# zhuwsh/ORB-SLAM2

Measured on AMD Instinct MI355X. Metric: frames/sec ORB extract+match, 1241x376 @1000 feats; bit-exact vs CPU, higher is better.
Workload: dtype u8; 1 GPU; KITTI-shape stereo 1241x376, nFeatures=1000/eye, 8 levels, FAST 20/7: extract(L)+extract(R)+ComputeStereoMatches; 1 frame = 1 stereo pair; images RESIDENT IN HBM when the timed region starts (kernel throughput: excludes PCIe; fed from pinned host memory the same path runs at config.host_fed_batched_frames_per_s -- the PCIe Gen5 x16 link, 0.96 MB per frame -- and one camera stream at config.host_fe; parallelism=1 independent camera-stream batches, one per GPU, ranks_seen=1, backend=none

## Files before the change

### orb-slam2_amd/csrc/orbx_stereo.hip

```cpp
#include "orbx_device.h"
#include <stdlib.h>
#include <algorithm>

struct StereoTabs {
    float sf[ORBX_MAX_LEVELS]; float isf[ORBX_MAX_LEVELS];
    unsigned long long reach_pk;
};

__device__ __forceinline__ int lvl_px(const uint8_t *img, int pitch, int w, int h, int x, int y)
{
    return img[(long long)reflect101(y, h) * pitch + reflect101(x, w)];
}

template <bool FOLD>
__device__ __forceinline__ void st_store(Published<float> u_right, Published<float> depth, Published<int> st_dist, long long og, float u, float z, int sad)
{
    if (FOLD) { u_right.put(og, u); depth.put(og, z); st_dist.put(og, sad); }
    else {
        u_right.plain_across_launches()[og] = u; depth.plain_across_launches()[og] = z; st_dist.plain_across_launches()[og] = sad;
    }
}

extern __shared__ __align__(16) int prep_smem[];

__global__ __launch_bounds__(256) void k_stereo_prep(const Geom *__restrict__ g, const orbx_keypoint *__restrict__ kR,
                                                     const int *__restrict__ nR, int cap, StereoTabs tabs,
                                                     int *__restrict__ row_off, uint4 *__restrict__ entries, int ent_cap)
{
    __shared__ int s_w[4];
    const int p = blockIdx.x, tid = threadIdx.x;
    const int rows = g->lv[0].h, n_r = min(nR[p], ent_cap);
    int *cnt = prep_smem, *cur = prep_smem + ((rows + 4) & ~3);
    const orbx_keypoint *kr = kR + (long long)p * cap;
    for (int i = tid; i < rows; i += 256) { cnt[i] = 0; cur[i] = 0; }
    __syncthreads();
    for (int ir = tid; ir < n_r; ir += 256) atomicAdd(&cnt[min(max((int)floorf(kr[ir].y), 0), rows - 1)], 1);
    __syncthreads();
    const int total = lds_excl_scan(cnt, rows, s_w);
    int *ro = row_off + (long long)p * (rows + 1);
    for (int i = tid; i < rows; i += 256) ro[i] = cnt[i];
    if (tid == 0) ro[rows] = total;
    uint4 *en = entries + (long long)p * ent_cap;
    for (int ir = tid; ir < n_r; ir += 256) {
        const orbx_keypoint q = kr[ir];
        const float y = q.y, r = 2.0f * tabs.sf[q.octave & (ORBX_MAX_LEVELS - 1)];
        const int maxr = min((int)ceilf(y + r), rows - 1), minr = max((int)floorf(y - r), 0);
        const int c = min(max((int)floorf(y), 0), rows - 1);
        en[cnt[c] + atomicAdd(&cur[c], 1)] = make_uint4((unsigned)ir | ((unsigned)q.octave << 16), __float_as_uint(q.x),
                                                        (unsigned)minr | ((unsigned)maxr << 16), 0u);
    }
}

__device__ __forceinline__ void hist_select(const int *hist, int k, int *sel, int *rem)
{
    const int lane = threadIdx.x;
    const int4 v = reinterpret_cast<const int4 *>(hist)[lane];
    const int s = v.x + v.y + v.z + v.w, inc = wave_incl_scan(s);
    const unsigned long long m = __ballot(inc > k);
    const int L = m ? __builtin_ctzll(m) : 63;
    if (lane == L) {
        int acc = inc - s, b = 0;
        if (acc + v.x > k) b = 0;
        else if (acc + v.x + v.y > k) { b = 1; acc += v.x; }
        else if (acc + v.x + v.y + v.z > k) { b = 2; acc += v.x + v.y; }
        else { b = 3; acc += v.x + v.y + v.z; }
        *sel = 4 * L + b; *rem = k - acc;
    }
}

__device__ __forceinline__ void stereo_cut(int n_l, long long o, Published<float> u_right, Published<float> depth, Published<int> st_dist)
{
    __shared__ __align__(16) int hist[256];
    __shared__ int s_sel, s_rem, s_cnt;
    const int tid = threadIdx.x;
    constexpr int K = 8;
    int d[K];
#pragma unroll
    for (int k = 0; k < K; k++) {
        const int i = tid + 256 * k;
        d[k] = i < n_l ? st_dist.get(o + i) : -1;
    }
    hist[tid] = 0;
    if (tid == 0) s_cnt = 0;
    __syncthreads();
    int local = 0;
#pragma unroll
    for (int k = 0; k < K; k++) if (d[k] >= 0) { atomicAdd(&hist[d[k] >> 8], 1); local++; }
    for (int i = tid + 256 * K; i < n_l; i += 256) {
        const int v = st_dist.get(o + i);
        if (v >= 0) { atomicAdd(&hist[v >> 8], 1); local++; }
    }
    if (local) atomicAdd(&s_cnt, local);
    __syncthreads();
    const int nvd = s_cnt;
    if (nvd == 0) return;
    if (tid < 64) hist_select(hist, nvd / 2, &s_sel, &s_rem);
    __syncthreads();
    const int hi = s_sel, rem = s_rem;
    __syncthreads();
    hist[tid] = 0;
    __syncthreads();
#pragma unroll
    for (int k = 0; k < K; k++) if (d[k] >= 0 && (d[k] >> 8) == hi) atomicAdd(&hist[d[k] & 255], 1);
    for (int i = tid + 256 * K; i < n_l; i += 256) {
        const int v = st_dist.get(o + i);
        if (v >= 0 && (v >> 8) == hi) atomicAdd(&hist[v & 255], 1);
    }
    __syncthreads();
    if (tid < 64) hist_select(hist, rem, &s_sel, &s_rem);
    __syncthreads();
    const float median = (float)((hi << 8) | s_sel);
    const float th_dist = 1.5f * 1.4f * median;
#pragma unroll
    for (int k = 0; k < K; k++)
        if (d[k] >= 0 && !((float)d[k] < th_dist)) { u_right.put(o + tid + 256 * k, -1.0f); depth.put(o + tid + 256 * k, -1.0f); }
    for (int i = tid + 256 * K; i < n_l; i += 256) {
        const int v = st_dist.get(o + i);
        if (v >= 0 && !((float)v < th_dist)) { u_right.put(o + i, -1.0f); depth.put(o + i, -1.0f); }
    }
}

#ifndef STX_G
#define STX_G 16
#endif
template <bool FOLD>
__global__ __launch_bounds__(256) __attribute__((amdgpu_waves_per_eu(8, 8))) void k_stereo(const Geom *__restrict__ g, PyrRef prL, PyrRef prR, int img_l0, int img_r0,
                                                const orbx_keypoint *__restrict__ kL, const uint32_t *__restrict__ dL,
                                                const int *__restrict__ nL, const orbx_keypoint *__restrict__ kR,
                                                const uint32_t *__restrict__ dR, const int *__restrict__ nR, int cap,
                                                float bf, float max_d, StereoTabs tabs, Published<float> u_right,
                                                Published<float> depth, Published<int> st_dist,
                                                const int *__restrict__ row_off, const uint4 *__restrict__ entries, int ent_cap, int reach,
                                                int *__restrict__ arrive, int kpw, int xmap_gx, int xmap_pairs)
{
    constexpr int SW_BYTES = 11 * 16 + 11 * 28 + 4;
    __shared__ __align__(16) uint8_t s_win[4 * ((SW_BYTES + 15) & ~15)];
    int p, bx;
    if (xmap_gx > 0) {
        const unsigned L = blockIdx.x, slot = L >> 3, per = (unsigned)xmap_gx * STX_G, grp = slot / per, rem = slot - grp * per;
        bx = (int)(rem / STX_G); p = (int)((grp * STX_G + rem % STX_G) * 8u + (L & 7u));
        if (p >= xmap_pairs) return;
    } else { p = blockIdx.y; bx = blockIdx.x; }
    const int lane = threadIdx.x & 63, sub = lane >> 4, sl = lane & 15;
    const int il_base = (bx * 4 + (threadIdx.x >> 6)) * kpw;
    const int n_l = nL[p];
    if (bx * 4 * kpw >= n_l) return;
    if (il_base < n_l) {
    const int il = il_base + sub;
    const bool have = il < n_l && sub < kpw;
    const long long ol = (long long)p * cap + (have ? il : il_base);
    const uint32_t *dr = dR + (long long)p * cap * 8;
    const orbx_keypoint kp = kL[ol];
    const int level_l = min(max(kp.octave, 0), g->nlevels - 1);
    const float vl = kp.y, ul = kp.x;
    const int n_rows = g->lv[0].h;
    const int row = (int)vl;
    const float min_u = ul - max_d, max_u = ul;
    const bool active = have && row >= 0 && row < n_rows && !(max_u < 0);
    unsigned mine = 0xFFFFFFFFu;
    float mine_x = 0.f;
    {
        uint32_t a[8];
#pragma unroll
        for (int i = 0; i < 8; i++) a[i] = dL[ol * 8 + i];
        const int *ro = row_off + (long long)p * (n_rows + 1);
        const uint4 *en = entries + (long long)p * ent_cap;
        const int rl = (int)((tabs.reach_pk >> (4 * level_l)) & 15ull);
        const int rch = rl == 15 ? reach : min(reach, rl);
        const int b0 = active ? ro[max(row - rch, 0)] : 0, e1 = active ? ro[min(row + rch, n_rows - 1) + 1] : 0;
        for (int base = b0; __any(base < e1); base += 16) {
            const int j = base + sl;
            if (j < e1) {
                const uint4 ent = en[j];
                const int ir = (int)(ent.x & 0xFFFFu), oct = (int)(short)(ent.x >> 16);
                const float qx = __uint_as_float(ent.y);
                const int minr = (int)(ent.z & 0xFFFFu), maxr = (int)(ent.z >> 16);
                if (row >= minr && row <= maxr && oct >= level_l - 1 && oct <= level_l + 1 && qx >= min_u && qx <= max_u) {
                    uint32_t bq[8];
                    const uint4 *src = reinterpret_cast<const uint4 *>(dr + (long long)ir * 8);
                    const uint4 v0 = src[0], v1 = src[1];
                    bq[0] = v0.x; bq[1] = v0.y; bq[2] = v0.z; bq[3] = v0.w;
                    bq[4] = v1.x; bq[5] = v1.y; bq[6] = v1.z; bq[7] = v1.w;
                    const int dist = hamming256(a, bq);
                    if (dist < 100) {
                        const unsigned key = ((unsigned)dist << 16) | (unsigned)ir;
                        if (key < mine) { mine = key; mine_x = qx; }
                    }
                }
            }
        }
    }
    const unsigned best_row = row16_min_u32(mine);
    const unsigned bx_row = row16_or_u32(mine == best_row && mine != 0xFFFFFFFFu ? __float_as_uint(mine_x) : 0u);
    for (int gk = 0; gk < kpw; gk++) {
        if (il_base + gk >= n_l) break;
        const unsigned best = (unsigned)__builtin_amdgcn_readlane((int)best_row, gk * 16);
        const int best_dist = best == 0xFFFFFFFFu ? 100 : (int)(best >> 16);
        const float ur0 = __uint_as_float((unsigned)__builtin_amdgcn_readlane((int)bx_row, gk * 16));
        const float kx = __uint_as_float((unsigned)__builtin_amdgcn_readlane((int)__float_as_uint(kp.x), gk * 16));
        const float ky = __uint_as_float((unsigned)__builtin_amdgcn_readlane((int)__float_as_uint(kp.y), gk * 16));
        const int lvl = __builtin_amdgcn_readlane(level_l, gk * 16);
        const long long og = (long long)p * cap + il_base + gk;
        if (!(best_dist < 75)) {
            if (lane == 0) st_store<FOLD>(u_right, depth, st_dist, og, -1.0f, -1.0f, -1);
            continue;
        }
        float out_u = -1.0f, out_z = -1.0f;
        int out_sad = -1;
        const float sfac = tabs.isf[lvl];
        const float sul = roundf(kx * sfac), svl = roundf(ky * sfac), sur0 = roundf(ur0 * sfac);
        const LevelGeom &LV = g->lv[lvl];
        const float iniu = sur0 + 5 - 5, endu = sur0 + 5 + 5 + 1;
        if (!(iniu < 0 || endu >= (float)LV.w)) {
            int pl, prr;
            const uint8_t *imL = orbx_level_ptr(prL, LV, lvl, img_l0 + p, &pl);
            const uint8_t *imR = orbx_level_ptr(prR, LV, lvl, img_r0 + p, &prr);
            const int cy = (int)svl, cxl = (int)sul;
            const int e0 = lane, e1 = lane + 64 < 121 ? lane + 64 : 60;
            const int dy0 = e0 / 11 - 5, dx0 = e0 % 11 - 5;
            const int dy1 = e1 / 11 - 5, dx1 = e1 % 11 - 5;
            const int cx0 = (int)sur0;
            int lc, il0, il1, r0[11], r1[11];
            const bool inside = cy - 5 >= 0 && cy + 5 < LV.h && cxl - 5 >= 0 && cxl + 5 < LV.w && cx0 - 10 >= 0 && cx0 + 10 < LV.w &&
                                ((((uintptr_t)imL | (uintptr_t)imR | (unsigned)pl | (unsigned)prr) & 3) == 0);
            if (inside) {
                uint8_t *wl = s_win + (threadIdx.x >> 6) * ((SW_BYTES + 15) & ~15), *wr = wl + 11 * 16;
                const int xla = (cxl - 5) & ~3, xra = (cx0 - 10) & ~3;
                uint32_t vr0, vr1 = 0, vlw = 0;
                {
                    const int rr = lane / 7, cc = lane - rr * 7;
                    const int xo_ = min(xra + 4 * cc, (prr - 4));
                    vr0 = *reinterpret_cast<const uint32_t *>(imR + (long long)(cy - 5 + rr) * prr + xo_);
                    if (lane < 13) {
                        const int i2 = lane + 64, r2 = i2 / 7, c2 = i2 - r2 * 7;
                        vr1 = *reinterpret_cast<const uint32_t *>(imR + (long long)(cy - 5 + r2) * prr + min(xra + 4 * c2, prr - 4));
                    }
                    if (lane < 44) {
                        const int r3 = lane >> 2, c3 = lane & 3;
                        vlw = *reinterpret_cast<const uint32_t *>(imL + (long long)(cy - 5 + r3) * pl + min(xla + 4 * c3, pl - 4));
                    }
                    __builtin_amdgcn_wave_barrier();
                    reinterpret_cast<uint32_t *>(wr)[lane] = vr0;
                    if (lane < 13) reinterpret_cast<uint32_t *>(wr)[lane + 64] = vr1;
                    if (lane < 44) reinterpret_cast<uint32_t *>(wl)[lane] = vlw;
                }
                __builtin_amdgcn_fence(__ATOMIC_RELEASE, "wavefront");
                __builtin_amdgcn_wave_barrier();
                const int ol_ = cxl - xla, or_ = cx0 - xra;
                typedef const volatile __attribute__((address_space(3))) uint8_t *lds_bytes;
                const lds_bytes vl_ = (lds_bytes)wl, vr_ = (lds_bytes)wr;
                lc = vl_[5 * 16 + ol_];
                il0 = vl_[(dy0 + 5) * 16 + ol_ + dx0];
                il1 = vl_[(dy1 + 5) * 16 + ol_ + dx1];
#pragma unroll
                for (int k = 0; k < 11; k++) {
                    r0[k] = vr_[(dy0 + 5) * 28 + or_ + dx0 + k - 5];
                    r1[k] = vr_[(dy1 + 5) * 28 + or_ + dx1 + k - 5];
                }
                asm volatile("" : "+v"(lc), "+v"(il0), "+v"(il1));
#pragma unroll
                for (int k = 0; k < 11; k++) asm volatile("" : "+v"(r0[k]), "+v"(r1[k]));
            } else {
                lc = lvl_px(imL, pl, LV.w, LV.h, cxl, cy);
                il0 = lvl_px(imL, pl, LV.w, LV.h, cxl + dx0, cy + dy0);
                il1 = lvl_px(imL, pl, LV.w, LV.h, cxl + dx1, cy + dy1);
#pragma unroll
                for (int k = 0; k < 11; k++) {
                    r0[k] = lvl_px(imR, prr, LV.w, LV.h, cx0 + dx0 + k - 5, cy + dy0);
                    r1[k] = lvl_px(imR, prr, LV.w, LV.h, cx0 + dx1 + k - 5, cy + dy1);
                }
            }
            int dists[11];
            unsigned lpk = (unsigned)il0 | ((unsigned)il1 << 16), lcc = (unsigned)lc * 0x00010001u;
            asm volatile("" : "+v"(lcc));
            auto shift_sad = [&](int k) -> unsigned {
                const unsigned rc = (unsigned)__builtin_amdgcn_readlane(r0[k], 60) * 0x00010001u;
                const unsigned rpk = (unsigned)r0[k] | ((unsigned)r1[k] << 16);
                return __builtin_amdgcn_sad_u16(lpk + rc, rpk + lcc, 0u);
            };
#pragma unroll
            for (int k = 0; k < 11; k += 2) {
                const unsigned sa = shift_sad(k);
                if (k + 1 < 11) {
                    const unsigned sb = shift_sad(k + 1);
                    const unsigned tot = (unsigned)wave_sum((int)(sa | (sb << 16)));
                    dists[k] = (int)(tot & 0xFFFFu);
                    dists[k + 1] = (int)(tot >> 16);
                } else {
                    dists[k] = wave_sum((int)sa);
                }
            }
            int best_sad = 0x7FFFFFFF, best_inc = 0;
#pragma unroll
            for (int k = 0; k < 11; k++)
                if (dists[k] < best_sad) { best_sad = dists[k]; best_inc = k - 5; }
            if (!(best_inc == -5 || best_inc == 5)) {
                float d1 = 0, d2 = 0, d3 = 0;
#pragma unroll
                for (int k = 1; k < 10; k++)
                    if (k == best_inc + 5) { d1 = (float)dists[k - 1]; d2 = (float)dists[k]; d3 = (float)dists[k + 1]; }
                const float delta = (d1 - d3) / (2.0f * (d1 + d3 - 2.0f * d2));
                if (!(delta < -1 || delta > 1)) {
                    float best_ur = tabs.sf[lvl] * ((float)sur0 + (float)best_inc + delta);
                    float disparity = kx - best_ur;
                    if (disparity >= 0 && disparity < max_d) {
                        if (disparity <= 0) { disparity = 0.01f; best_ur = (float)((double)kx - 0.01); }
                        out_z = bf / disparity;
                        out_u = best_ur;
                        out_sad = best_sad;
                    }
                }
            }
        }
        if (lane == 0) st_store<FOLD>(u_right, depth, st_dist, og, out_u, out_z, out_sad);
    }
    }
    if (!FOLD) return;
    __shared__ int s_last;
    publish_drain();
    __syncthreads();
    if (threadIdx.x == 0) {
        const int nwg = (n_l + 4 * kpw - 1) / (4 * kpw);
        const int old = publish_arrive(&arrive[p]);
        s_last = old == nwg - 1;
        if (old == nwg - 1) __hip_atomic_store(&arrive[p], 0, __ATOMIC_RELAXED, __HIP_MEMORY_SCOPE_AGENT);
    }
    __syncthreads();
    if (!s_last) return;
    stereo_cut(n_l, (long long)p * cap, u_right, depth, st_dist);
}

__global__ __launch_bounds__(256) void k_stereo_cut(const int *__restrict__ nL, int cap, Published<float> u_right,
                                                    Published<float> depth, Published<int> st_dist)
{
    stereo_cut(nL[blockIdx.x], (long long)blockIdx.x * cap, u_right, depth, st_dist);
}

static int same_geometry(const orbx_extractor *L, const orbx_extractor *R)
{
    if (L->nlevels != R->nlevels || L->geom.w != R->geom.w || L->geom.h != R->geom.h || L->geom.w == 0) return 0;
    for (int i = 0; i < L->nlevels; i++) if (L->sf[i] != R->sf[i]) return 0;
    return 1;
}

extern "C" int orbx_stereo_row_table_available(const orbx_extractor *R, const void *d_kR, int img_r0, int batch, int cap)
{
    return R && d_kR && img_r0 >= 0 && batch >= 1 && R->d_rt_off && R->rt_kps && cap == R->rt_cap && img_r0 + batch <= R->rt_batch &&
           (const char *)d_kR == (const char *)R->rt_kps + (size_t)img_r0 * cap * sizeof(orbx_keypoint);
}

extern "C" int orbx_stereo_match_batch_device(orbx_extractor *L, int img_l0, orbx_extractor *R, int img_r0, int batch,
                                              const void *d_kL, const void *d_dL, const void *d_nL,
                                              const void *d_kR, const void *d_dR, const void *d_nR, int cap,
                                              float bf, float min_z, void *d_u_right, void *d_depth, int row_table, void *stream)
{
    if (row_table != ORBX_ROWTAB_FROM_KEYPOINTS && row_table != ORBX_ROWTAB_OF_EXTRACTION) { orbx_set_error("row_table: unknown source %d", row_table); return ORBX_E_INVALID; }
    if (!L || !R || !d_kL || !d_dL || !d_nL || !d_kR || !d_dR || !d_nR || !d_u_right || !d_depth || batch < 1 || cap < 1 ||
        img_l0 < 0 || img_r0 < 0 || img_l0 + batch > L->last_batch || img_r0 + batch > R->last_batch || !(min_z > 0)) {
        orbx_set_error("orbx_stereo_match_batch_device: invalid argument");
        return ORBX_E_INVALID;
    }
    if (L->device != R->device || !same_geometry(L, R)) {
        orbx_set_error("left and right extractors differ in device, image size or scale tables");
        return ORBX_E_INVALID;
    }
    if (cap >= 65536) { orbx_set_error("cap must be < 65536"); return ORBX_E_INVALID; }
    ORBX_HIP(orbx_use_device(L->device));
    hipStream_t s = stream ? (hipStream_t)stream : L->stream;
    const size_t need = (size_t)batch * cap * sizeof(int);
    if (need > L->st_cap || !L->d_st_dist) {
        ORBX_HIP(hipStreamSynchronize(s));
        { const int qrc = orbx_quiesce(L); if (qrc) return qrc; }
        { const int erc = ensure(&L->d_st_dist, &L->st_cap, need); if (erc) return erc; }
    }
    StereoTabs tabs;
    tabs.reach_pk = 0;
    for (int i = 0; i < ORBX_MAX_LEVELS; i++) {
        tabs.sf[i] = L->sf[i]; tabs.isf[i] = L->isf[i];
        const int rl = (int)ceilf(2.0f * L->sf[std::min(i + 1, L->nlevels - 1)]) + 1;
        tabs.reach_pk |= (unsigned long long)std::min(rl, 15) << (4 * i);
    }
    const int rows = L->geom.lv[0].h;
    const int ent_cap = cap;
    const int reach = (int)ceilf(2.0f * L->sf[L->nlevels - 1]) + 1;
    void *d_row_off, *d_entries;
    int row_ent_cap = ent_cap;
    const bool by_product = row_table == ORBX_ROWTAB_OF_EXTRACTION;
    if (by_product && !orbx_stereo_row_table_available(R, d_kR, img_r0, batch, cap)) {
        orbx_set_error("ORBX_ROWTAB_OF_EXTRACTION: the right handle's last extraction left no row table for this keypoint buffer / capacity / image range");
        return ORBX_E_INVALID;
    }
    if (by_product) {
        d_row_off = R->d_rt_off + (size_t)img_r0 * (rows + 1);
        d_entries = R->d_rt_entries + (size_t)img_r0 * R->rt_ent_cap * sizeof(uint4);
        row_ent_cap = R->rt_ent_cap;
    } else {
        int rc;
        if ((rc = orbx_scratch(L, 7, (size_t)batch * (rows + 1) * sizeof(int), &d_row_off))) return rc;
        const size_t need_e = (size_t)batch * ent_cap * sizeof(uint4);
        if (need_e > L->st_ent_cap || !L->d_st_entries) {
            ORBX_HIP(hipStreamSynchronize(s));
            { const int qrc = orbx_quiesce(L); if (qrc) return qrc; }
            if ((rc = ensure(&L->d_st_entries, &L->st_ent_cap, need_e))) return rc;
        }
        d_entries = L->d_st_entries;
    }
    PyrRef pl, pr;
    pl.img0 = L->last_img0; pl.img0_stride = (long long)L->last_img_stride; pl.img0_pitch = (int)L->last_pitch;
    pl.pyr = L->d_pyr; pl.pyr_stride = L->geom.pyr_bytes;
    pr.img0 = R->last_img0; pr.img0_stride = (long long)R->last_img_stride; pr.img0_pitch = (int)R->last_pitch;
    pr.pyr = R->d_pyr; pr.pyr_stride = R->geom.pyr_bytes;
    { int urc = orbx_use_stream(L, s); if (urc) return urc; if (R != L && (urc = orbx_use_stream(R, s))) return urc; }
    const float max_d = bf / min_z;
    if (!L->d_st_arrive) {
        ORBX_HIP(hipMalloc((void **)&L->d_st_arrive, (size_t)L->max_batch * sizeof(int)));
        ORBX_HIP(hipMemsetAsync(L->d_st_arrive, 0, (size_t)L->max_batch * sizeof(int), s));
    }
    orbx_prof_begin(L, ORBX_STAGE_STEREO, s);
    if (!by_product)
        hipLaunchKernelGGL(k_stereo_prep, dim3(batch), dim3(256), (size_t)2 * ((rows + 4) & ~3) * sizeof(int), s, L->d_geom,
                           (const orbx_keypoint *)d_kR, (const int *)d_nR, cap, tabs, (int *)d_row_off, (uint4 *)d_entries, ent_cap);
    const int kpw_forced = L->stereo_kpw_forced;
    const int kpw = kpw_forced ? kpw_forced : (long long)batch * cap <= 2560 ? 1 : 4;
    const bool fold = kpw == 1;
    const int gx = (cap + 4 * kpw - 1) / (4 * kpw);
#ifdef STX_NOXMAP
    const bool xmap = false;
#else
    const bool xmap = !fold && batch >= 16 && (long long)gx * ((batch + 8 * STX_G - 1) / (8 * STX_G)) * 8 * STX_G < (1ll << 30);
#endif
    const dim3 grid = xmap ? dim3((unsigned)(gx * ((batch + 8 * STX_G - 1) / (8 * STX_G)) * 8 * STX_G)) : dim3(gx, batch);
    L->last_forms[7] = kpw; L->last_forms[8] = xmap;
    hipLaunchKernelGGL((fold ? k_stereo<true> : k_stereo<false>), grid, dim3(256), 0, s, L->d_geom, pl, pr, img_l0, img_r0,
                       (const orbx_keypoint *)d_kL, (const uint32_t *)d_dL, (const int *)d_nL,
                       (const orbx_keypoint *)d_kR, (const uint32_t *)d_dR, (const int *)d_nR, cap, bf, max_d, tabs,
                       Published<float>((float *)d_u_right), Published<float>((float *)d_depth), Published<int>(L->d_st_dist), (const int *)d_row_off, (const uint4 *)d_entries, row_ent_cap, reach,
                       L->d_st_arrive, kpw, xmap ? gx : 0, batch);
    if (!fold) hipLaunchKernelGGL(k_stereo_cut, dim3(batch), dim3(256), 0, s, (const int *)d_nL, cap, Published<float>((float *)d_u_right), Published<float>((float *)d_depth), Published<int>(L->d_st_dist));
    orbx_prof_end(L, s);
    ORBX_HIP(hipGetLastError());
    return ORBX_OK;
}

extern "C" int orbx_stereo_match(orbx_extractor *L, orbx_extractor *R,
                                 const orbx_keypoint *kL, const uint8_t *dL, int nL,
                                 const orbx_keypoint *kR, const uint8_t *dR, int nR,
                                 float bf, float min_z, float *u_right, float *depth)
{
    if (!L || !R || nL < 0 || nR < 0 || (nL && (!kL || !dL || !u_right || !depth)) || (nR && (!kR || !dR))) {
        orbx_set_error("orbx_stereo_match: invalid argument");
        return ORBX_E_INVALID;
    }
    if (nL == 0) return ORBX_OK;
    for (int i = 0; i < nL; i++)
        if (kL[i].octave < 0 || kL[i].octave >= L->nlevels) { orbx_set_error("left keypoint %d: octave %d out of range", i, kL[i].octave); return ORBX_E_INVALID; }
    for (int i = 0; i < nR; i++)
        if (kR[i].octave < 0 || kR[i].octave >= L->nlevels) { orbx_set_error("right keypoint %d: octave %d out of range", i, kR[i].octave); return ORBX_E_INVALID; }
    if (!L->last_img0 || !R->last_img0) { orbx_set_error("run orbx_extract on both eyes first"); return ORBX_E_INVALID; }
    ORBX_HIP(orbx_use_device(L->device));
    ORBX_HIP(hipStreamSynchronize(R->stream));
    const int cap = nL > nR ? nL : (nR > 0 ? nR : 1);
    void *bkL, *bdL, *bkR, *bdR, *bn, *bu, *bz;
    int rc;
    if ((rc = orbx_scratch(L, 0, sizeof(orbx_keypoint) * cap, &bkL)) || (rc = orbx_scratch(L, 1, 32 * (size_t)cap, &bdL)) ||
        (rc = orbx_scratch(L, 2, sizeof(orbx_keypoint) * cap, &bkR)) || (rc = orbx_scratch(L, 3, 32 * (size_t)cap, &bdR)) ||
        (rc = orbx_scratch(L, 4, 2 * sizeof(int), &bn)) || (rc = orbx_scratch(L, 5, 4 * (size_t)cap, &bu)) ||
        (rc = orbx_scratch(L, 6, 4 * (size_t)cap, &bz)))
        return rc;
    const int counts[2] = { nL, nR };
    hipStream_t s = L->stream;
    ORBX_HIP(hipMemcpyAsync(bkL, kL, sizeof(orbx_keypoint) * nL, hipMemcpyHostToDevice, s));
    ORBX_HIP(hipMemcpyAsync(bdL, dL, 32 * (size_t)nL, hipMemcpyHostToDevice, s));
    if (nR) {
        ORBX_HIP(hipMemcpyAsync(bkR, kR, sizeof(orbx_keypoint) * nR, hipMemcpyHostToDevice, s));
        ORBX_HIP(hipMemcpyAsync(bdR, dR, 32 * (size_t)nR, hipMemcpyHostToDevice, s));
    }
    ORBX_HIP(hipMemcpyAsync(bn, counts, sizeof counts, hipMemcpyHostToDevice, s));
    L->prof_chain = false;
    rc = orbx_stereo_match_batch_device(L, 0, R, 0, 1, bkL, bdL, bn, bkR, bdR, (int *)bn + 1, cap, bf, min_z, bu, bz, ORBX_ROWTAB_FROM_KEYPOINTS, s);
    if (rc) return rc;
    ORBX_HIP(hipMemcpyAsync(u_right, bu, 4 * (size_t)nL, hipMemcpyDeviceToHost, s));
    ORBX_HIP(hipMemcpyAsync(depth, bz, 4 * (size_t)nL, hipMemcpyDeviceToHost, s));
    ORBX_HIP(hipStreamSynchronize(s));
    return ORBX_OK;
}
```

Baseline: 159,500 frames/s.

## Prefetch stereo SAD windows for all per-wave keypoints via async global-to-LDS loads

Result: no change. 159,800 frames/s (median of 5 runs) (+0.2%).

```diff
diff --git a/orb-slam2_amd/csrc/orbx_stereo.hip b/orb-slam2_amd/csrc/orbx_stereo.hip
--- a/orb-slam2_amd/csrc/orbx_stereo.hip
+++ b/orb-slam2_amd/csrc/orbx_stereo.hip
@@ -123,6 +123,8 @@
 #ifndef STX_G
 #define STX_G 16
 #endif
+constexpr int STX_SLOT = (11 * 16 + 11 * 28 + 4 + 15) & ~15;
+extern __shared__ __align__(16) uint8_t stereo_smem[];
 template <bool FOLD>
 __global__ __launch_bounds__(256) __attribute__((amdgpu_waves_per_eu(8, 8))) void k_stereo(const Geom *__restrict__ g, PyrRef prL, PyrRef prR, int img_l0, int img_r0,
                                                 const orbx_keypoint *__restrict__ kL, const uint32_t *__restrict__ dL,
@@ -131,10 +133,10 @@
                                                 float bf, float max_d, StereoTabs tabs, Published<float> u_right,
                                                 Published<float> depth, Published<int> st_dist,
                                                 const int *__restrict__ row_off, const uint4 *__restrict__ entries, int ent_cap, int reach,
-                                                int *__restrict__ arrive, int kpw, int xmap_gx, int xmap_pairs)
-{
-    constexpr int SW_BYTES = 11 * 16 + 11 * 28 + 4;
-    __shared__ __align__(16) uint8_t s_win[4 * ((SW_BYTES + 15) & ~15)];
+                                                int *__restrict__ arrive, int kpw_arg, int xmap_gx, int xmap_pairs)
+{
+    constexpr int kpw = FOLD ? 1 : 4;
+    (void)kpw_arg;
     int p, bx;
     if (xmap_gx > 0) {
         const unsigned L = blockIdx.x, slot = L >> 3, per = (unsigned)xmap_gx * STX_G, grp = slot / per, rem = slot - grp * per;
@@ -168,85 +170,119 @@
         const int rl = (int)((tabs.reach_pk >> (4 * level_l)) & 15ull);
         const int rch = rl == 15 ? reach : min(reach, rl);
         const int b0 = active ? ro[max(row - rch, 0)] : 0, e1 = active ? ro[min(row + rch, n_rows - 1) + 1] : 0;
-        for (int base = b0; __any(base < e1); base += 16) {
-            const int j = base + sl;
-            if (j < e1) {
-                const uint4 ent = en[j];
-                const int ir = (int)(ent.x & 0xFFFFu), oct = (int)(short)(ent.x >> 16);
-                const float qx = __uint_as_float(ent.y);
-                const int minr = (int)(ent.z & 0xFFFFu), maxr = (int)(ent.z >> 16);
-                if (row >= minr && row <= maxr && oct >= level_l - 1 && oct <= level_l + 1 && qx >= min_u && qx <= max_u) {
-                    uint32_t bq[8];
-                    const uint4 *src = reinterpret_cast<const uint4 *>(dr + (long long)ir * 8);
-                    const uint4 v0 = src[0], v1 = src[1];
-                    bq[0] = v0.x; bq[1] = v0.y; bq[2] = v0.z; bq[3] = v0.w;
-                    bq[4] = v1.x; bq[5] = v1.y; bq[6] = v1.z; bq[7] = v1.w;
-                    const int dist = hamming256(a, bq);
-                    if (dist < 100) {
-                        const unsigned key = ((unsigned)dist << 16) | (unsigned)ir;
-                        if (key < mine) { mine = key; mine_x = qx; }
-                    }
-                }
+        for (int base = b0; __any(base < e1); base += 32) {
+            const int j0 = base + sl, j1 = j0 + 16;
+            uint4 ent0 = make_uint4(0u, 0u, 0u, 0u), ent1 = ent0;
+            if (j0 < e1) ent0 = en[j0];
+            if (j1 < e1) ent1 = en[j1];
+            const int ir0 = (int)(ent0.x & 0xFFFFu), oct0 = (int)(short)(ent0.x >> 16), ir1 = (int)(ent1.x & 0xFFFFu), oct1 = (int)(short)(ent1.x >> 16);
+            const float qx0 = __uint_as_float(ent0.y), qx1 = __uint_as_float(ent1.y);
+            const int minr0 = (int)(ent0.z & 0xFFFFu), maxr0 = (int)(ent0.z >> 16), minr1 = (int)(ent1.z & 0xFFFFu), maxr1 = (int)(ent1.z >> 16);
+            const bool ok0 = j0 < e1 && row >= minr0 && row <= maxr0 && oct0 >= level_l - 1 && oct0 <= level_l + 1 && qx0 >= min_u && qx0 <= max_u;
+            const bool ok1 = j1 < e1 && row >= minr1 && row <= maxr1 && oct1 >= level_l - 1 && oct1 <= level_l + 1 && qx1 >= min_u && qx1 <= max_u;
+            uint4 p0 = make_uint4(0u, 0u, 0u, 0u), p1 = p0, q0 = p0, q1 = p0;
+            if (ok0) { const uint4 *src = reinterpret_cast<const uint4 *>(dr + (long long)ir0 * 8); p0 = src[0]; p1 = src[1]; }
+            if (ok1) { const uint4 *src = reinterpret_cast<const uint4 *>(dr + (long long)ir1 * 8); q0 = src[0]; q1 = src[1]; }
+            const uint32_t bp[8] = { p0.x, p0.y, p0.z, p0.w, p1.x, p1.y, p1.z, p1.w }, bq[8] = { q0.x, q0.y, q0.z, q0.w, q1.x, q1.y, q1.z, q1.w };
+            const int dist0 = hamming256(a, bp), dist1 = hamming256(a, bq);
+            if (ok0 && dist0 < 100) {
+                const unsigned key = ((unsigned)dist0 << 16) | (unsigned)ir0;
+                if (key < mine) { mine = key; mine_x = qx0; }
+            }
+            if (ok1 && dist1 < 100) {
+                const unsigned key = ((unsigned)dist1 << 16) | (unsigned)ir1;
+                if (key < mine) { mine = key; mine_x = qx1; }
             }
         }
     }
     const unsigned best_row = row16_min_u32(mine);
     const unsigned bx_row = row16_or_u32(mine == best_row && mine != 0xFFFFFFFFu ? __float_as_uint(mine_x) : 0u);
+    struct Fine {
+        bool match, range, inside;
+        int lvl, w, h, cy, cxl, cx0;
+        float kx, sur0;
+    };
+    struct FineImgs { const uint8_t *imL, *imR; int pl, prr; };
+    auto imgs_of = [&](int lvl) -> FineImgs {
+        FineImgs m;
+        const LevelGeom &LV = g->lv[lvl];
+        m.imL = orbx_level_ptr(prL, LV, lvl, img_l0 + p, &m.pl);
+        m.imR = orbx_level_ptr(prR, LV, lvl, img_r0 + p, &m.prr);
+        return m;
+    };
+    auto fine_of = [&](int gk) -> Fine {
+        Fine f;
+        const unsigned best = (unsigned)__builtin_amdgcn_readlane((int)best_row, gk * 16);
+        const int best_dist = best == 0xFFFFFFFFu ? 100 : (int)(best >> 16);
+        f.match = best_dist < 75;
+        const float ur0 = __uint_as_float((unsigned)__builtin_amdgcn_readlane((int)bx_row, gk * 16));
+        f.kx = __uint_as_float((unsigned)__builtin_amdgcn_readlane((int)__float_as_uint(kp.x), gk * 16));
+        const float ky = __uint_as_float((unsigned)__builtin_amdgcn_readlane((int)__float_as_uint(kp.y), gk * 16));
+        f.lvl = __builtin_amdgcn_readlane(level_l, gk * 16);
+        const float sfac = tabs.isf[f.lvl];
+        const float sul = roundf(f.kx * sfac), svl = roundf(ky * sfac);
+        f.sur0 = roundf(ur0 * sfac);
+        const LevelGeom &LV = g->lv[f.lvl];
+        f.w = LV.w; f.h = LV.h;
+        const float iniu = f.sur0 + 5 - 5, endu = f.sur0 + 5 + 5 + 1;
+        f.range = !(iniu < 0 || endu >= (float)LV.w);
+        const FineImgs m = imgs_of(f.lvl);
+        f.cy = (int)svl; f.cxl = (int)sul; f.cx0 = (int)f.sur0;
+        f.inside = f.cy - 5 >= 0 && f.cy + 5 < LV.h && f.cxl - 5 >= 0 && f.cxl + 5 < LV.w && f.cx0 - 10 >= 0 && f.cx0 + 10 < LV.w &&
+                   ((((uintptr_t)m.imL | (uintptr_t)m.imR | (unsigned)m.pl | (unsigned)m.prr) & 3) == 0);
+        return f;
+    };
+    uint8_t *const slots = stereo_smem + __builtin_amdgcn_readfirstlane((int)(threadIdx.x >> 6)) * kpw * STX_SLOT;
+    int st_pk = 0;
+    float st_sur0 = 0.f;
+#pragma unroll
     for (int gk = 0; gk < kpw; gk++) {
         if (il_base + gk >= n_l) break;
-        const unsigned best = (unsigned)__builtin_amdgcn_readlane((int)best_row, gk * 16);
-        const int best_dist = best == 0xFFFFFFFFu ? 100 : (int)(best >> 16);
-        const float ur0 = __uint_as_float((unsigned)__builtin_amdgcn_readlane((int)bx_row, gk * 16));
-        const float kx = __uint_as_float((unsigned)__builtin_amdgcn_readlane((int)__float_as_uint(kp.x), gk * 16));
-        const float ky = __uint_as_float((unsigned)__builtin_amdgcn_readlane((int)__float_as_uint(kp.y), gk * 16));
-        const int lvl = __builtin_amdgcn_readlane(level_l, gk * 16);
-        const long long og = (long long)p * cap + il_base + gk;
-        if (!(best_dist < 75)) {
-            if (lane == 0) st_store<FOLD>(u_right, depth, st_dist, og, -1.0f, -1.0f, -1);
-            continue;
+        if (!(((unsigned)__builtin_amdgcn_readlane((int)best_row, gk * 16) >> 16) < 75u)) continue;
+        const Fine f = fine_of(gk);
+        const bool staged = f.match && f.range && f.inside;
+        const int pk = (int)f.match | (int)f.range << 1 | (int)staged << 2 | ((f.cxl - 5) & 3) << 3 | ((f.cx0 - 10) & 3) << 5;
+        if (lane == gk) { st_pk = pk; st_sur0 = f.sur0; }
+        if (staged) {
+            const FineImgs m = imgs_of(f.lvl);
+            uint8_t *wl = slots + gk * STX_SLOT, *wr = wl + 11 * 16;
+            const int xla = (f.cxl - 5) & ~3, xra = (f.cx0 - 10) & ~3;
+            const int rr = lane / 7, cc = lane - rr * 7;
+            __builtin_amdgcn_global_load_lds(reinterpret_cast<const uint32_t *>(m.imR + (long long)(f.cy - 5 + rr) * m.prr + min(xra + 4 * cc, m.prr - 4)),
+                                             reinterpret_cast<uint32_t *>(wr), 4, 0, 0);
+            if (lane < 13) {
+                const int i2 = lane + 64, r2 = i2 / 7, c2 = i2 - r2 * 7;
+                __builtin_amdgcn_global_load_lds(reinterpret_cast<const uint32_t *>(m.imR + (long long)(f.cy - 5 + r2) * m.prr + min(xra + 4 * c2, m.prr - 4)),
+                                                 reinterpret_cast<uint32_t *>(wr + 256), 4, 0, 0);
+            }
+            if (lane < 44) {
+                const int r3 = lane >> 2, c3 = lane & 3;
+                __builtin_amdgcn_global_load_lds(reinterpret_cast<const uint32_t *>(m.imL + (long long)(f.cy - 5 + r3) * m.pl + min(xla + 4 * c3, m.pl - 4)),
+                                                 reinterpret_cast<uint32_t *>(wl), 4, 0, 0);
+            }
         }
+    }
+    asm volatile("s_waitcnt vmcnt(0)" ::: "memory");
+    __builtin_amdgcn_wave_barrier();
+    float res_u = -1.0f, res_z = -1.0f;
+    int res_sad = -1;
+    for (int gk = 0; gk < kpw; gk++) {
+        if (il_base + gk >= n_l) break;
+        const int pk = __builtin_amdgcn_readlane(st_pk, gk);
+        if (!(pk & 1)) continue;
         float out_u = -1.0f, out_z = -1.0f;
         int out_sad = -1;
-        const float sfac = tabs.isf[lvl];
-        const float sul = roundf(kx * sfac), svl = roundf(ky * sfac), sur0 = roundf(ur0 * sfac);
-        const LevelGeom &LV = g->lv[lvl];
-        const float iniu = sur0 + 5 - 5, endu = sur0 + 5 + 5 + 1;
-        if (!(iniu < 0 || endu >= (float)LV.w)) {
-            int pl, prr;
-            const uint8_t *imL = orbx_level_ptr(prL, LV, lvl, img_l0 + p, &pl);
-            const uint8_t *imR = orbx_level_ptr(prR, LV, lvl, img_r0 + p, &prr);
-            const int cy = (int)svl, cxl = (int)sul;
+        const int lvl = __builtin_amdgcn_readlane(level_l, gk * 16);
+        const float kx = __uint_as_float((unsigned)__builtin_amdgcn_readlane((int)__float_as_uint(kp.x), gk * 16));
+        const float sur0 = __uint_as_float((unsigned)__builtin_amdgcn_readlane((int)__float_as_uint(st_sur0), gk));
+        if (pk & 2) {
             const int e0 = lane, e1 = lane + 64 < 121 ? lane + 64 : 60;
             const int dy0 = e0 / 11 - 5, dx0 = e0 % 11 - 5;
             const int dy1 = e1 / 11 - 5, dx1 = e1 % 11 - 5;
-            const int cx0 = (int)sur0;
             int lc, il0, il1, r0[11], r1[11];
-            const bool inside = cy - 5 >= 0 && cy + 5 < LV.h && cxl - 5 >= 0 && cxl + 5 < LV.w && cx0 - 10 >= 0 && cx0 + 10 < LV.w &&
-                                ((((uintptr_t)imL | (uintptr_t)imR | (unsigned)pl | (unsigned)prr) & 3) == 0);
-            if (inside) {
-                uint8_t *wl = s_win + (threadIdx.x >> 6) * ((SW_BYTES + 15) & ~15), *wr = wl + 11 * 16;
-                const int xla = (cxl - 5) & ~3, xra = (cx0 - 10) & ~3;
-                uint32_t vr0, vr1 = 0, vlw = 0;
-                {
-                    const int rr = lane / 7, cc = lane - rr * 7;
-                    const int xo_ = min(xra + 4 * cc, (prr - 4));
-                    vr0 = *reinterpret_cast<const uint32_t *>(imR + (long long)(cy - 5 + rr) * prr + xo_);
-                    if (lane < 13) {
-                        const int i2 = lane + 64, r2 = i2 / 7, c2 = i2 - r2 * 7;
-                        vr1 = *reinterpret_cast<const uint32_t *>(imR + (long long)(cy - 5 + r2) * prr + min(xra + 4 * c2, prr - 4));
-                    }
-                    if (lane < 44) {
-                        const int r3 = lane >> 2, c3 = lane & 3;
-                        vlw = *reinterpret_cast<const uint32_t *>(imL + (long long)(cy - 5 + r3) * pl + min(xla + 4 * c3, pl - 4));
-                    }
-                    __builtin_amdgcn_wave_barrier();
-                    reinterpret_cast<uint32_t *>(wr)[lane] = vr0;
-                    if (lane < 13) reinterpret_cast<uint32_t *>(wr)[lane + 64] = vr1;
-                    if (lane < 44) reinterpret_cast<uint32_t *>(wl)[lane] = vlw;
-                }
-                __builtin_amdgcn_fence(__ATOMIC_RELEASE, "wavefront");
-                __builtin_amdgcn_wave_barrier();
-                const int ol_ = cxl - xla, or_ = cx0 - xra;
+            if (pk & 4) {
+                const uint8_t *wl = slots + gk * STX_SLOT, *wr = wl + 11 * 16;
+                const int ol_ = 5 + ((pk >> 3) & 3), or_ = 10 + ((pk >> 5) & 3);
                 typedef const volatile __attribute__((address_space(3))) uint8_t *lds_bytes;
                 const lds_bytes vl_ = (lds_bytes)wl, vr_ = (lds_bytes)wr;
                 lc = vl_[5 * 16 + ol_];
@@ -261,13 +297,17 @@
 #pragma unroll
                 for (int k = 0; k < 11; k++) asm volatile("" : "+v"(r0[k]), "+v"(r1[k]));
             } else {
-                lc = lvl_px(imL, pl, LV.w, LV.h, cxl, cy);
-                il0 = lvl_px(imL, pl, LV.w, LV.h, cxl + dx0, cy + dy0);
-                il1 = lvl_px(imL, pl, LV.w, LV.h, cxl + dx1, cy + dy1);
+                const Fine f = fine_of(gk);
+                const FineImgs m = imgs_of(lvl);
+                const uint8_t *imL = m.imL, *imR = m.imR;
+                const int pl = m.pl, prr = m.prr, lw = f.w, lh = f.h, cy = f.cy, cxl = f.cxl, cx0 = f.cx0;
+                lc = lvl_px(imL, pl, lw, lh, cxl, cy);
+                il0 = lvl_px(imL, pl, lw, lh, cxl + dx0, cy + dy0);
+                il1 = lvl_px(imL, pl, lw, lh, cxl + dx1, cy + dy1);
 #pragma unroll
                 for (int k = 0; k < 11; k++) {
-                    r0[k] = lvl_px(imR, prr, LV.w, LV.h, cx0 + dx0 + k - 5, cy + dy0);
-                    r1[k] = lvl_px(imR, prr, LV.w, LV.h, cx0 + dx1 + k - 5, cy + dy1);
+                    r0[k] = lvl_px(imR, prr, lw, lh, cx0 + dx0 + k - 5, cy + dy0);
+                    r1[k] = lvl_px(imR, prr, lw, lh, cx0 + dx1 + k - 5, cy + dy1);
                 }
             }
             int dists[11];
@@ -312,8 +352,9 @@
                 }
             }
         }
-        if (lane == 0) st_store<FOLD>(u_right, depth, st_dist, og, out_u, out_z, out_sad);
-    }
+        if (lane == gk) { res_u = out_u; res_z = out_z; res_sad = out_sad; }
+    }
+    if (lane < kpw && il_base + lane < n_l) st_store<FOLD>(u_right, depth, st_dist, (long long)p * cap + il_base + lane, res_u, res_z, res_sad);
     }
     if (!FOLD) return;
     __shared__ int s_last;
@@ -431,7 +472,7 @@
 #endif
     const dim3 grid = xmap ? dim3((unsigned)(gx * ((batch + 8 * STX_G - 1) / (8 * STX_G)) * 8 * STX_G)) : dim3(gx, batch);
     L->last_forms[7] = kpw; L->last_forms[8] = xmap;
-    hipLaunchKernelGGL((fold ? k_stereo<true> : k_stereo<false>), grid, dim3(256), 0, s, L->d_geom, pl, pr, img_l0, img_r0,
+    hipLaunchKernelGGL((fold ? k_stereo<true> : k_stereo<false>), grid, dim3(256), (size_t)4 * kpw * STX_SLOT, s, L->d_geom, pl, pr, img_l0, img_r0,
                        (const orbx_keypoint *)d_kL, (const uint32_t *)d_dL, (const int *)d_nL,
                        (const orbx_keypoint *)d_kR, (const uint32_t *)d_dR, (const int *)d_nR, cap, bf, max_d, tabs,
                        Published<float>((float *)d_u_right), Published<float>((float *)d_depth), Published<int>(L->d_st_dist), (const int *)d_row_off, (const uint4 *)d_entries, row_ent_cap, reach,
```
